# scholarsmate/omega-match

Measured on NVIDIA B200. Metric: haystack_throughput, higher is better.
Workload: dtype u8

## Files before the change

### omega_match_b200/csrc/api.cpp

```cpp
#include <unistd.h>

#include <cstdio>
#include <cstdlib>
#include <cstring>
#include <exception>
#include <string>
#include <thread>

#include "../../include/olm_b200.h"
#include "engine.h"
#include "host_util.h"
#include "multi.h"
#include "store.h"

#ifndef OLM_B200_VERSION
#define OLM_B200_VERSION "0.1.0"
#endif

struct olm_cuda_comm {
  olm::Comm *comm = nullptr;
};

struct omega_list_matcher_struct {
  olm::Engine *engine = nullptr;
// ... 328 lines not shown
int olm_cuda_comm_unique_id(void *id, size_t id_bytes) { return olm::comm_unique_id(id, id_bytes); }

olm_cuda_comm_t *olm_cuda_comm_create(const omega_list_matcher_t *m, const void *id, int rank, int world) {
  if (!m || !m->engine || m->multi) return nullptr;
  olm::Comm *c = olm::comm_create(m->engine, id, rank, world);
  if (!c) return nullptr;
  auto *h = new olm_cuda_comm();
  h->comm = c;
  return h;
}

int olm_cuda_comm_destroy(olm_cuda_comm_t *c) {
  if (!c) return -1;
  olm::comm_destroy(c->comm);
  delete c;
  return 0;
}

int olm_cuda_gather_records(olm_cuda_comm_t *c, const void *dev_records, uint64_t count, int root, int no_overlap,
                            olm_cuda_results_t *out) {
  if (!c || !c->comm) return -1;
  return olm::comm_gather(c->comm, dev_records, count, root, no_overlap != 0, out);
}

int olm_store_inspect(const char *compiled_file, olm_store_info_t *out) {
  if (!compiled_file || !out) return -1;
  size_t n = 0;
  uint8_t *f = olm::map_whole_file(compiled_file, &n, false);
  if (!f) return -1;
  olm::StoreView v;
  const std::string err = olm::parse_store(f, n, &v);
  int rc = -1;
  if (err.empty()) try {
    olm::StagedStore s;
    olm::FilterBudget b;
    const std::string e2 = olm::stage_store(v, b, &s);
    olm::StagedStats ss;
    if (e2.empty() && olm::check_staged_store(v, s) == 0 && olm::stage_stats(v, &ss).empty()) {
      out->flags = v.hdr.flags;
      out->smallest = v.hdr.smallest;
      out->largest = v.hdr.largest;
      out->stored_patterns = v.hdr.stored_patterns;
      out->table_size = v.hdr.table_size;
      out->occupied_buckets = v.hdr.occupied;
      out->len1 = v.n1;
      out->len2 = v.n2;
      out->len3 = v.n3;
      out->len4 = v.n4;
      out->store_bytes = v.hdr.store_bytes;
      out->file_bytes = n;
      out->gram_keys = s.n_keys;
      out->key_bytes = s.params.key_bytes;
      out->key_buckets = s.params.key_mask + 1;
      out->g4_bits = s.params.g4_words * 32;
      out->class_run = s.params.cls.run;
      out->class_and_mask = s.params.cls.and_mask;
      out->class_ranges = s.params.cls.n_ranges;
      for (int i = 0; i < 2; ++i) {
        out->class_lo[i] = s.params.cls.lo[i];
        out->class_hi[i] = s.params.cls.hi[i];
      }
      rc = 0;
    } else {
      std::fprintf(stderr, "libomega_match(b200): %s: %s\n", compiled_file, e2.empty() ? "self check failed" : e2.c_str());
    }
  } catch (const std::exception &ex) {
    std::fprintf(stderr, "libomega_match(b200): %s: malformed store (%s)\n", compiled_file, ex.what());
    rc = -1;
  } else {
    std::fprintf(stderr, "libomega_match(b200): %s: %s\n", compiled_file, err.c_str());
  }
  olm::unmap(f, n);
  return rc;
}

}
```

### omega_match_b200/csrc/device_tables.h

```cpp
#pragma once
#include <cstdint>
#include <vector_types.h>

namespace olm {

struct alignas(16) Slot {
  uint32_t w0;
  uint32_t w1;
  uint32_t meta;
  uint32_t ref;
};
constexpr uint32_t kSlotShort4 = 1u << 31;
constexpr uint32_t kSlotMulti = 1u << 30;
constexpr uint32_t kSlotValueMask = (1u << 30) - 1;

struct alignas(16) Rec {
  uint32_t w0;
  uint32_t len;
  uint32_t store_off;
  uint32_t w1;
};

constexpr uint32_t kHashMul = 0x9E3779B1u;
constexpr uint32_t kHashMul2 = 0x85EBCA6Bu;

#if defined(__CUDACC__)
__host__ __device__
#endif
inline uint32_t key_hash(uint32_t gram, uint32_t tail) { return (gram * kHashMul) ^ (tail * kHashMul2); }

struct ByteClass {
  uint32_t run = 0;
  uint32_t and_mask = 0;
  uint32_t n_ranges = 0;
  uint32_t lo[2] = {0, 0}, hi[2] = {0, 0};
  uint32_t and4 = 0, addlo[2] = {0, 0}, addhi[2] = {0, 0};
};

struct DeviceStore {
  const uint4 *keys = nullptr;
  const Slot *slots = nullptr;
  const Rec *recs = nullptr;
  const uint8_t *store = nullptr;
  const uint32_t *g4 = nullptr;
  const uint32_t *p23 = nullptr;
  const uint32_t *set3 = nullptr;
  const uint32_t *bitmap2 = nullptr;
  uint32_t bitmap1[8] = {0};
  uint32_t key_shift = 32;
  uint32_t key_mask = 0;
  uint32_t empty_key = 0;
  uint32_t key_bytes = 4;
  uint32_t tail_mask = 0;
  uint32_t g4_shift = 32, g4_words = 0;
  uint32_t p23_and = 0, p23_mul = 1, p23_shift = 32, p23_words = 0;
  const uint32_t *sx = nullptr;
  uint32_t sx_words = 0, sx3_shift = 32;
  uint32_t set3_mask = 0;
  uint32_t n_long = 0, n1 = 0, n2 = 0, n3 = 0, n4 = 0;
  uint32_t smallest = 0, largest = 0;
  uint32_t flags = 0;
  uint32_t max_recs = 0;
  uint32_t coop = 0;
  ByteClass cls;
};
#ifndef OLM_COOP_MIN
#define OLM_COOP_MIN 4
#endif
constexpr uint32_t kCoopMinRecs = OLM_COOP_MIN;

}
```

### omega_match_b200/csrc/engine.cu

```cuda
#include "engine.h"

#include <algorithm>
#include <atomic>
#include <condition_variable>
#include <cstdio>
#include <cstdlib>
#include <cstring>
#include <memory>
#include <mutex>
#include <thread>
#include <vector>

#include <cuda_runtime.h>

#include "filters.cuh"
#include "format.cuh"
#include "scan.cuh"
#include "stats.cuh"
#include "transform.cuh"

namespace olm {

namespace {

// ... 90 lines not shown
  uint64_t host_span = 0;
  omega_match_stats_t span_acc{};
};

namespace {
size_t seg_event_for(const EngineImpl &E, uint64_t bytes) {
  if (E.seg_events.size() <= 1 || E.seg_bytes == 0 || bytes == 0) return 0;
  return std::min<size_t>(E.seg_events.size() - 1, size_t((bytes - 1) / E.seg_bytes));
}
int wait_segment(EngineImpl &E, size_t idx) {
  Stager &S = E.stager;
  for (size_t j = std::min(E.seg_waited, idx); j <= idx; ++j) {
    if (S.active) {
      std::unique_lock<std::mutex> lk(S.mu);
      S.cv.wait(lk, [&] { return S.recorded[j] || S.failed.load(); });
      if (S.failed.load()) return -1;
    }
    if (cudaStreamWaitEvent(E.stream, E.seg_events[j], 0) != cudaSuccess) return -1;
  }
  E.seg_waited = std::max(E.seg_waited, idx + 1);
  return 0;
}
}

Engine *Engine::create(const uint8_t *file, size_t size, int device, std::string *err) {
  auto fail = [&](const std::string &m) -> Engine * {
    if (err) *err = m;
    return nullptr;
  };
  StoreView view;
  std::string e = parse_store(file, size, &view);
  if (!e.empty()) return fail(e);

  int ndev = 0;
  if (cudaGetDeviceCount(&ndev) != cudaSuccess || ndev == 0)
    return fail("no CUDA device: this library has no CPU matching path");
  if (device < 0 || device >= ndev) return fail("CUDA device index out of range");
  if (cudaSetDevice(device) != cudaSuccess) return fail("cudaSetDevice failed");
  cudaDeviceProp prop;
  if (cudaGetDeviceProperties(&prop, device) != cudaSuccess) return fail("cudaGetDeviceProperties failed");
  if (prop.major < 10) return fail("this build contains sm_100a code only (needs a B200 class GPU)");

  auto *impl = new EngineImpl();
  Engine *eng = new Engine();
  eng->impl_ = impl;
  impl->device = device;
  impl->sms = prop.multiProcessorCount;
  impl->smem_limit = prop.sharedMemPerBlockOptin;
  impl->hdr = view.hdr;

  StagedStore staged;
  FilterBudget budget;
  const bool has_p23 = view.n1 || view.n2 || view.n3;
  budget.g4_max_log2 = (has_p23 || (view.hdr.flags & kFlagAnyTransform)) ? 19 : OLM_G4_MAX_LOG2;
  budget.p23_max_log2 = 18;
  e = stage_store(view, budget, &staged);
  if (e.empty() && check_staged_store(view, staged) != 0) e = "internal error: staged store failed its self check";
  if (!e.empty()) {
    delete eng;
    return fail(e);
  }
  impl->has_short_234 = view.n2 || view.n3 || view.n4;
  impl->ds = staged.params;
  bool ok = true;
  ok = ok && upload(impl->d_keys, staged.keys, &impl->ds.keys) == 0;
  ok = ok && upload(impl->d_slots, staged.slots, &impl->ds.slots) == 0;
  ok = ok && upload(impl->d_recs, staged.recs, &impl->ds.recs) == 0;
  ok = ok && upload(impl->d_store, staged.store, &impl->ds.store) == 0;
  ok = ok && upload(impl->d_g4, staged.g4, &impl->ds.g4) == 0;
  ok = ok && upload(impl->d_p23, staged.p23, &impl->ds.p23) == 0;
  if (impl->ds.sx_words) ok = ok && upload(impl->d_sx, staged.sx, &impl->ds.sx) == 0;
  ok = ok && upload(impl->d_set3, staged.set3, &impl->ds.set3) == 0;
  ok = ok && upload(impl->d_bitmap2, staged.bitmap2, &impl->ds.bitmap2) == 0;
  if (const char *sp = std::getenv("OLM_HOST_SPAN_BYTES")) {
    const unsigned long long v = std::strtoull(sp, nullptr, 10);
    impl->host_span = (v + kWindowBytes - 1) / kWindowBytes * kWindowBytes;
  }
  {
    StagedStats ss;
    e = stage_stats(view, &ss);
    if (!e.empty()) {
      delete eng;
      return fail(e);
    }
    impl->stats.bloom_mask = ss.bloom_mask;
    impl->stats.map_shift = ss.map_shift;
    impl->stats.map_mask = ss.map_mask;
    impl->stats.largest = view.hdr.largest;
    ok = ok && upload(impl->d_bloom, ss.bloom, &impl->stats.bloom) == 0;
    ok = ok && upload(impl->d_smap, ss.map, &impl->stats.map) == 0;
    ok = ok && upload(impl->d_slens, ss.lens, &impl->stats.lens) == 0;
  }
  ok = ok && cudaStreamCreateWithFlags(&impl->stream, cudaStreamNonBlocking) == cudaSuccess;
  ok = ok && cudaStreamCreateWithFlags(&impl->copy_stream, cudaStreamNonBlocking) == cudaSuccess;
  for (auto &ev : impl->ev) ok = ok && cudaEventCreate(&ev) == cudaSuccess;
  ok = ok && scan_configure(impl->smem_limit) == cudaSuccess;
  impl->geo = scan_pick_geometry(impl->ds, impl->smem_limit);
  if (impl->ds.sx_words) {
    DeviceStore plain = impl->ds;
    plain.sx_words = 0;
    const ScanGeometry g0 = scan_pick_geometry(plain, impl->smem_limit);
    const char *env = std::getenv("OLM_SHORT_LOOK");
    const bool plain_store = !(impl->hdr.flags & kFlagAnyTransform) && !impl->ds.coop;
    const bool weak_p23 = plain_store && (env ? std::atoi(env) != 0 : impl->ds.p23_mul == 1);
    const bool room = impl->geo.stages != 0 && (impl->geo.stages >= g0.stages || impl->geo.stages >= 8) &&
                      impl->geo.chunk_cap >= std::min<uint32_t>(g0.chunk_cap, 256);
    if (!weak_p23 || !room) {
// ... 642 lines not shown
```

### omega_match_b200/csrc/scan.cu

```cuda
#include "scan.cuh"

#include <cstddef>
#include <cstdio>

#include "olm_classes.h"
#include "olm_format.h"
#include "scan_device.cuh"

namespace olm {

namespace {

using namespace dev;

#ifndef OLM_FAST_UNROLL
#define OLM_FAST_UNROLL 2
#endif
#ifndef OLM_GRAB
#define OLM_GRAB 1
#endif
constexpr uint32_t kGrab = OLM_GRAB;
static_assert(kGrab >= 1 && kTileChunks % kGrab == 0, "a grab stays inside one tile");
#ifndef OLM_TICKET_BATCH
#define OLM_TICKET_BATCH 4
// ... 164 lines not shown
      c = T.tail;
    }
    if (fl & kWordBoundary) {
      if (L == 1) {
        if (inside && is_word_byte(c)) return false;
      } else if (is_word_byte(c)) {
        return false;
      }
    }
    if ((fl & kWordSuffix) && inside && is_word_byte(c)) return false;
    if ((fl & kLineEnd) && inside && !is_line_end_byte(c)) return false;
    return true;
  }

  static constexpr uint32_t kNoSlot = 0xFFFFFFFFu;
  static constexpr uint32_t kCoopMin = kCoopMinRecs;
  struct Probe {
    uint32_t tpos, gram, bucket, flags;
    uint4 kb;
  };

  __device__ __forceinline__ void probe_issue(const TileCtx &T, bool valid, uint32_t tpos, bool cand_g, bool cand_p,
                                              Probe &pr) const {
    pr.tpos = tpos;
    pr.flags = 0;
    pr.gram = 0;
    pr.bucket = 0;
    pr.kb = make_uint4(0, 0, 0, 0);
    uint32_t bad_start = 0;
    if (!valid) return;
    const uint32_t q = T.sb32 + kTilePre + tpos;
    if (fl & (kWordBoundary | kWordPrefix | kLineStart)) {
      const bool at0 = T.first && tpos == 0;
      const uint32_t prev = lds8(q - 1);
      if (fl & kWordBoundary) {
        const bool cw = is_word_byte(lds8(q));
        const bool pw = at0 ? false : is_word_byte(prev);
        if (cw == pw) return;
      }
      bool bad = (fl & kWordPrefix) && !at0 && is_word_byte(prev);
      bad = bad || ((fl & kLineStart) && !at0 && !is_line_end_byte(prev));
      if (bad) {
        if (!((fl & kCountAll) && (cand_p || (cand_g && P.st.n4)))) return;
        bad_start = 8u;
      }
    }
    const uint32_t gram = __byte_perm(lds_le32(q), 0, 0x0123);
    if (SX && cand_p) cand_p = short_look(gram);
    pr.flags = 1u | (cand_p ? 4u : 0u) | bad_start;
    if (HAS_G4 && cand_g && T.rem0 - tpos >= P.st.key_bytes) {
      const uint32_t h = key_hash(gram, P.st.tail_mask ? lds_le32(q + 4) & P.st.tail_mask : 0u);
      pr.gram = h;
      if (HAS_CLS) {
        const uint32_t b = h >> P.st.g4_shift;
        if (!((g4s[b >> 5] >> (b & 31)) & 1u)) return;
      }
      pr.flags |= 2u;
      pr.bucket = h >> P.st.key_shift;
      pr.kb = __ldg(P.st.keys + pr.bucket);
    }
  }

  __device__ __forceinline__ bool probe_key(const Probe &pr, uint32_t *slot) const {
    *slot = kNoSlot;
    if (!(pr.flags & 1u)) return false;
    if (HAS_G4 && (pr.flags & 2u)) {
      const uint32_t gram = pr.gram;
      uint4 kb = pr.kb;
      uint32_t bucket = pr.bucket;
      int place;
      while (true) {
        place = kb.x == gram ? 0 : kb.y == gram ? 1 : kb.z == gram ? 2 : kb.w == gram ? 3 : -1;
        if (place >= 0 || kb.w == P.st.empty_key) break;
        bucket = (bucket + 1) & P.st.key_mask;
        kb = __ldg(P.st.keys + bucket);
      }
      if (place >= 0) *slot = 4 * bucket + (uint32_t)place;
    }
    return *slot != kNoSlot || (HAS_P23 && (pr.flags & 4u));
  }

  template <typename Emit>
  __device__ __forceinline__ void verify(const TileCtx &T, uint32_t tpos, uint32_t slot, const uint4 &s_in, bool cand_p,
                                         bool bad_start, bool coop_done, bool emitted, Emit &&emit) const {
    const uint32_t rem = T.rem0 - tpos;
    const uint32_t q = T.sb32 + kTilePre + tpos;
    const bool longest = fl & kLongestOnly;
    const bool count_all = fl & kCountAll;

    if (HAS_G4 && slot != kNoSlot) {
      const uint4 s = COOP ? s_in : __ldg(reinterpret_cast<const uint4 *>(P.st.slots + slot));
      const uint32_t meta = s.z;
      if (meta != 0 && bad_start) {
        if (meta & kSlotShort4) n_miss += stat_inc;
      } else if (meta != 0) {
        const unsigned long long hay = ((unsigned long long)lds_le32(q + 4) << 32) | lds_le32(q);
        if (meta & kSlotValueMask) {
          n_hits += stat_inc;
          n_long_hits += stat_inc;
        }
        auto head_equal = [&](uint32_t len, uint32_t w0, uint32_t w1) {
          const uint32_t drop = len >= 8 ? 0u : (8u - len) * 8u;
          return ((hay ^ (((unsigned long long)w1 << 32) | w0)) << drop) == 0;
        };
        if (meta & kSlotMulti) {
          const uint32_t cnt = (coop_done || !next_bytes_ok(hay, s.x, s.y)) ? 0u : meta & kSlotValueMask;
          for (uint32_t j = 0; j < cnt; ++j) {
// ... 73 lines not shown
            n_hits += stat_inc;
          } else {
            n_miss += stat_inc;
          }
        }
      }
    }
  }

  static __device__ __forceinline__ uint32_t gather4(uint32_t m) { return __umulhi(m, 0x02040810u) & 0xFu; }

  __device__ __forceinline__ uint32_t class_runs16(const uint4 &v, const uint2 &nx) const {
    const ByteClass &c = P.st.cls;
    const uint32_t w[6] = {v.x, v.y, v.z, v.w, nx.x, nx.y};
    const uint32_t and4 = c.and4, lo0 = c.addlo[0], hi0 = c.addhi[0];
    uint32_t a = 0;
    if (c.n_ranges > 1) {
      const uint32_t lo1 = c.addlo[1], hi1 = c.addhi[1];
#pragma unroll
      for (int i = 0; i < 6; ++i) {
        const uint32_t t = w[i] & and4;
        const uint32_t in = ((t + lo0) & ~(t + hi0)) | ((t + lo1) & ~(t + hi1));
        a |= gather4(in & ~w[i] & 0x80808080u) << (4 * i);
      }
    } else {
#pragma unroll
      for (int i = 0; i < 6; ++i) {
        const uint32_t t = w[i] & and4;
        a |= gather4((t + lo0) & ~(t + hi0) & ~w[i] & 0x80808080u) << (4 * i);
      }
    }
    a &= a >> 1;
    a &= a >> 2;
    a &= a >> (c.run - 4);
    return a & 0xFFFFu;
  }
  __device__ __forceinline__ void stage1(const TileCtx &T, uint32_t lpos, uint32_t &cg, uint32_t &cp) const {
    const uint32_t src = T.sb32 + kTilePre + lpos;
    const uint4 v = lds128(src);
    cg = 0;
    cp = 0;
    if (HAS_CLS) {
      cg = class_runs16(v, lds64(src + 16));
      return;
    }
    const uint2 w45 = lds64(src + 16);
    const uint32_t w[6] = {v.x, v.y, v.z, v.w, w45.x, w45.y};
    const uint32_t tmask = P.st.tail_mask;
#pragma unroll
    for (int k = 0; k < 16; ++k) {
      const uint32_t gram = __byte_perm(w[k >> 2], w[(k >> 2) + 1], 0x0123u + 0x1111u * (k & 3));
      if (HAS_G4) {
        const uint32_t tail = __byte_perm(w[(k >> 2) + 1], w[(k >> 2) + 2 > 5 ? 5 : (k >> 2) + 2], 0x3210u + 0x1111u * (k & 3));
        const uint32_t b = key_hash(gram, tail & tmask) >> P.st.g4_shift;
        cg |= ((g4s[b >> 5] >> (b & 31)) & 1u) << k;
      }
      if (HAS_P23) {
        const uint32_t b = ((gram & P.st.p23_and) * P.st.p23_mul) >> P.st.p23_shift;
        cp |= ((p23s[b >> 5] >> (b & 31)) & 1u) << k;
      }
    }
  }

  template <int MODE>
  __device__ __forceinline__ uint32_t verify_batch(const TileCtx &T, uint32_t q2, uint32_t n, uint32_t lane,
                                                   uint32_t stage, uint32_t used, uint32_t cap, uint32_t cbase,
                                                   unsigned long long out_base, uint32_t *overflow) const {
    bool mine = lane < n;
    const unsigned long long ent = mine ? lds64u(q2 + 8u * lane) : 0ull;
    const uint32_t slot = (uint32_t)ent, hi = (uint32_t)(ent >> 32);
    const uint32_t tpos = hi & 0xFFFFu;
    const bool cand_p = (hi >> 16) & 1u, bad_start = (hi >> 17) & 1u;
    uint32_t at = 0, tot = 0, skip = 0;
    const uint32_t keep = stat_inc;
    bool again;
    uint4 s = make_uint4(0, 0, 0, 0);
    if (COOP && HAS_G4 && mine && slot != kNoSlot) s = __ldg(reinterpret_cast<const uint4 *>(P.st.slots + slot));
    do {
      uint32_t cnt = 0, m0 = 0, m1 = 0, m2 = 0, m3 = 0;
      auto emit = [&](uint32_t len) {
        const uint32_t j = cnt - skip;
        if (j == 0) m0 = len;
        else if (j == 1) m1 = len;
        else if (j == 2) m2 = len;
        else if (j == 3) m3 = len;
        ++cnt;
      };
      bool coop = false, emitted0 = false;
      if (COOP && HAS_G4) {
        coop = mine && s.z != 0 && !bad_start && (s.z & kSlotMulti) && (s.z & kSlotValueMask) >= kCoopMin;
        if (coop) {
          const uint32_t mq = T.sb32 + kTilePre + tpos;
          coop = next_bytes_ok(((unsigned long long)lds_le32(mq + 4) << 32) | lds_le32(mq), s.x, s.y);
        }
        uint32_t todo = __ballot_sync(kFull, coop);
        while (todo) {
          const uint32_t src = __ffs(todo) - 1;
          todo &= todo - 1;
          const uint32_t o_tpos = __shfl_sync(kFull, tpos, src), o_first = __shfl_sync(kFull, s.w, src);
          const uint32_t o_cnt = __shfl_sync(kFull, s.z, src) & kSlotValueMask;
          const uint32_t oq = T.sb32 + kTilePre + o_tpos, o_rem = T.rem0 - o_tpos;
          const unsigned long long hay = ((unsigned long long)lds_le32(oq + 4) << 32) | lds_le32(oq);
          uint32_t ncmp = 0;
          for (uint32_t base = 0; base < o_cnt; base += 32) {
            const bool valid = base + lane < o_cnt;
            uint4 r = make_uint4(0, 0, 0, 0);
            if (valid) r = __ldg(reinterpret_cast<const uint4 *>(P.st.recs + o_first + base + lane));
// ... 102 lines not shown
    for (uint32_t base = 0; base < total; base += 32 * kProbeUnroll) {
      Probe pr[kProbeUnroll];
#pragma unroll
      for (int u = 0; u < kProbeUnroll; ++u) {
        const uint32_t idx = base + u * 32 + lane;
        const bool ok = idx < total;
        const uint32_t e = ok ? lds16(q1 + 2u * idx) : 0u;
        probe_issue(T, ok, cbase + (e & 511u), (e >> 9) & 1u, (e >> 10) & 1u, pr[u]);
      }
#pragma unroll
      for (int u = 0; u < kProbeUnroll; ++u) {
        if (base + u * 32 >= total) break;
        uint32_t slot;
        const bool want = probe_key(pr[u], &slot);
        const uint32_t bal = __ballot_sync(kFull, want);
        if (want)
          sts64u(q2 + 8u * (q2n + __popc(bal & lt)),
                 ((unsigned long long)(pr[u].tpos | ((pr[u].flags & 12u) << 14)) << 32) | slot);
        q2n += __popc(bal);
      }
      __syncwarp();
      const bool last = base + 32 * kProbeUnroll >= total;
      while (q2n >= 32 || (last && q2n)) {
        const uint32_t nb = q2n < 32 ? q2n : 32;
        found += verify_batch<MODE>(T, q2, nb, lane, stage, found, cap, cbase, out_base, overflow);
        const uint32_t rest = q2n - nb;
        const unsigned long long mv0 = lane < rest ? lds64u(q2 + 8u * (32 + lane)) : 0ull;
        const unsigned long long mv1 = 32 + lane < rest ? lds64u(q2 + 8u * (64 + lane)) : 0ull;
        __syncwarp();
        if (lane < rest) sts64u(q2 + 8u * lane, mv0);
        if (32 + lane < rest) sts64u(q2 + 8u * (32 + lane), mv1);
        __syncwarp();
        q2n = rest;
      }
    }
    __syncwarp();
    return found;
  }

  template <int MODE, bool PRED>
  __device__ __forceinline__ uint32_t scan_chunk_fast(const TileCtx &T, uint32_t sb_off, uint32_t g4_off,
                                                      uint32_t p23_off, uint32_t q1_off, uint32_t q2_off,
                                                      uint32_t cbase, uint32_t lane, uint32_t stage, uint32_t cap,
                                                      unsigned long long out_base, uint32_t *overflow) const {
    const uint32_t lpos = cbase + lane * 16;
    const uint32_t src = sb_off + kTilePre + lpos;
    const uint4 v = lds128(src);
    uint32_t cand = 0, cp = 0;
    if (HAS_CLS) {
      cand = class_runs16(v, lds64(src + 16));
    } else {
      const uint2 w45 = lds64(src + 16);
      const uint32_t w[6] = {v.x, v.y, v.z, v.w, w45.x, w45.y};
      const uint32_t sh = P.st.g4_shift, tmask = P.st.tail_mask;
      const uint32_t pand = P.st.p23_and, pmul = P.st.p23_mul, psh = P.st.p23_shift;
#pragma unroll
      for (int k = 0; k < 16; ++k) {
        const uint32_t gram = __byte_perm(w[k >> 2], w[(k >> 2) + 1], 0x0123u + 0x1111u * (k & 3));
        if (HAS_G4) {
          uint32_t hk = gram * kHashMul;
          if (!HAS_P23) {
            const uint32_t tail = __byte_perm(w[(k >> 2) + 1], w[(k >> 2) + 2 > 5 ? 5 : (k >> 2) + 2], 0x3210u + 0x1111u * (k & 3));
            hk ^= (tail & tmask) * kHashMul2;
          }
          const uint32_t b = hk >> sh;
          const uint32_t word = lds32(g4_off + ((b >> 5) << 2));
          cand |= ((word >> (b & 31)) & 1u) << k;
        }
        if (HAS_P23) {
          const uint32_t b = ((gram & pand) * pmul) >> psh;
          const uint32_t word = lds32(p23_off + ((b >> 5) << 2));
          cp |= ((word >> (b & 31)) & 1u) << k;
        }
      }
    }
    const uint32_t rem_c = T.rem0 - cbase;
    const uint32_t kbytes = P.st.key_bytes;
    if (rem_c < (uint32_t)kChunkBytes + 8u) {
      const uint32_t fit = rem_c >= kbytes ? rem_c - kbytes + 1u : 0u, lrel = lane * 16;
      cand &= lrel >= fit ? 0u : (fit - lrel >= 16u ? 0xFFFFu : ((1u << (fit - lrel)) - 1u));
    }
    const uint32_t cg = cand;
    cand |= cp;
    if (lpos + 16 > T.nscan) cand &= lpos >= T.nscan ? 0u : ((1u << (T.nscan - lpos)) - 1u);
    const uint32_t cnt = __popc(cand);
    uint32_t incl = cnt;
#pragma unroll
    for (int d = 1; d < 32; d <<= 1) {
      const uint32_t t = __shfl_up_sync(kFull, incl, d);
      if (lane >= (uint32_t)d) incl += t;
    }
    const uint32_t total = __shfl_sync(kFull, incl, 31);
    if (total == 0) return 0;
    {
      uint32_t qa = q1_off + 2u * (incl - cnt);
      if (__any_sync(kFull, cnt > 4)) {
        const uint32_t eb = lane * 16;
#pragma unroll
        for (int k = 0; k < 16; ++k)
          if ((cand >> k) & 1u) {
            uint32_t ent = eb + k;
            if (HAS_P23) ent |= (((cg >> k) & 1u) << 9) | (((cp >> k) & 1u) << 10);
            sts16(qa, ent);
            qa += 2;
          }
      } else {
        const uint32_t eb = lane * 16;
        while (cand) {
          const uint32_t k = __ffs(cand) - 1;
          uint32_t ent = eb + k;
          if (HAS_P23) ent |= (((cg >> k) & 1u) << 9) | (((cp >> k) & 1u) << 10);
          sts16(qa, ent);
          cand &= cand - 1;
          qa += 2;
        }
      }
    }
    __syncwarp();
    const uint32_t q2 = q2_off;
    const uint32_t lt = (1u << lane) - 1u;
    const uint32_t tile_off = sb_off + kTilePre + cbase;
    const uint32_t key_shift = P.st.key_shift, g4_shift = P.st.g4_shift, empty = P.st.empty_key;
    const uint4 *keys = P.st.keys;
    const uint32_t tmask = P.st.tail_mask;
    uint32_t found = 0, q2n = 0;
    constexpr int U = OLM_FAST_UNROLL;
    for (uint32_t base = 0; base < total; base += 32 * U) {
      uint32_t e[U], gram[U], bucket[U];
      bool pass[U], shortc[U];
      uint4 kb[U];
#pragma unroll
      for (int u = 0; u < U; ++u) {
        const uint32_t idx = base + u * 32 + lane;
        pass[u] = idx < total;
        e[u] = pass[u] ? lds16(q1_off + 2u * idx) : 0u;
        shortc[u] = false;
        if (HAS_P23) {
          shortc[u] = (e[u] >> 10) & 1u;
          pass[u] = pass[u] && ((e[u] >> 9) & 1u);
          e[u] &= 511u;
        }
        const uint32_t a = tile_off + e[u], a4 = a & ~3u, sh8 = a << 3;
        const uint32_t x0 = lds32(a4), x1 = lds32(a4 + 4);
        const uint32_t gbe = __byte_perm(__funnelshift_r(x0, x1, sh8), 0, 0x0123);
        if (PRED) {
          const bool at0 = T.first && cbase + e[u] == 0;
          const uint32_t prev = lds8(a - 1), cur = gbe >> 24;
          bool ok = true;
          if (fl & kWordBoundary) ok = is_word_byte(cur) != (at0 ? false : is_word_byte(prev));
          if ((fl & kWordPrefix) && !at0 && is_word_byte(prev)) ok = false;
          if ((fl & kLineStart) && !at0 && !is_line_end_byte(prev)) ok = false;
          pass[u] = pass[u] && ok;
          shortc[u] = shortc[u] && ok;
        }
        if (SX && __any_sync(kFull, shortc[u])) shortc[u] = shortc[u] && short_look(gbe);
        uint32_t h = gbe * kHashMul;
        if (tmask) h ^= (__funnelshift_r(x1, lds32(a4 + 8), sh8) & tmask) * kHashMul2;
        gram[u] = h;
        if (HAS_CLS && !OLM_CLS_SKIP_BITMAP) {
          const uint32_t b = h >> g4_shift;
          const uint32_t word = lds32(g4_off + ((b >> 5) << 2));
          pass[u] = pass[u] && ((word >> (b & 31)) & 1u);
        }
        bucket[u] = h >> key_shift;
        if (HAS_G4 && pass[u]) kb[u] = ld_keys(keys + bucket[u]);
      }
      static_assert(U == 2, "Q2 holds 31 + 2 x 32 entries");
#pragma unroll
      for (int u = 0; u < U; ++u) {
        if (u > 0 && base + u * 32 >= total) break;
        const uint32_t g = gram[u];
        bool hit = HAS_G4 && pass[u] && (kb[u].x == g || kb[u].y == g || kb[u].z == g || kb[u].w == g);
        const bool more = HAS_G4 && pass[u] && !hit && kb[u].w != empty;
        if (!__any_sync(kFull, hit || more || (HAS_P23 && shortc[u]))) continue;
        if (HAS_G4 && __any_sync(kFull, more)) {
          while (pass[u] && !hit && kb[u].w != empty) {
            bucket[u] = (bucket[u] + 1) & P.st.key_mask;
            kb[u] = ld_keys(keys + bucket[u]);
            hit = kb[u].x == g || kb[u].y == g || kb[u].z == g || kb[u].w == g;
          }
        }
        const bool want = hit || (HAS_P23 && shortc[u]);
        const uint32_t bal = __ballot_sync(kFull, want);
        if (!bal) continue;
        const uint32_t place = kb[u].y == g ? 1u : kb[u].z == g ? 2u : kb[u].w == g ? 3u : 0u;
        const uint32_t slot = hit ? 4u * bucket[u] + place : kNoSlot;
        const uint32_t hi32 = (cbase + e[u]) | (HAS_P23 && shortc[u] ? 0x10000u : 0u);
        if (want) sts64u(q2 + 8u * (q2n + __popc(bal & lt)), ((unsigned long long)hi32 << 32) | slot);
        q2n += __popc(bal);
      }
      __syncwarp();
      const bool last = base + 32 * U >= total;
      while (q2n >= 32 || (last && q2n)) {
        const uint32_t nb = q2n < 32 ? q2n : 32;
        found += verify_batch<MODE>(T, q2, nb, lane, stage, found, cap, cbase, out_base, overflow);
        const uint32_t rest = q2n - nb;
        const unsigned long long mv0 = lane < rest ? lds64u(q2 + 8u * (32 + lane)) : 0ull;
        const unsigned long long mv1 = 32 + lane < rest ? lds64u(q2 + 8u * (64 + lane)) : 0ull;
        __syncwarp();
        if (lane < rest) sts64u(q2 + 8u * lane, mv0);
        if (32 + lane < rest) sts64u(q2 + 8u * (32 + lane), mv1);
        __syncwarp();
        q2n = rest;
      }
    }
    __syncwarp();
    return found;
  }

  __device__ __forceinline__ void flush_stats(uint32_t lane) const {
    unsigned long long h = n_hits, mi = n_miss, cm = n_cmp, lh = n_long_hits;
#pragma unroll
    for (int d = 16; d > 0; d >>= 1) {
// ... 256 lines not shown
                        priv32, sc.xf32, lane, true, T);
      __syncwarp();
      if (lane == 0) mbar_arrive32(scanned32 + 8u * s);
      cb = 0;
      work = work && T.nscan != 0;
    } else {
      tile_ctx(I, stage_sb, T);
    }
    if (work) {
      if (FAST)
        n = sc.template scan_chunk_fast<kStageMode, FAST == 2>(T, T.sb32, g4_32, p23_32, q1_32, q2_32, cb, lane, stage32, cap, 0, &ovf);
      else
        n = sc.template scan_chunk<kStageMode>(T, cb, lane, stage32, cap, q1_32, q2_32, 0, &ovf);
    }
    __syncwarp();
    if (!priv_mode && lane == 0) mbar_arrive32(scanned32 + 8u * s);
    ovf = __any_sync(kFull, ovf != 0);
    ChunkDesc d;
    d.count = n;
    d.temp_index = 0;
    if (ovf) {
      d.count = n | kChunkOverflow;
      if (lane == 0) *reinterpret_cast<volatile unsigned int *>(P.redo_flag) = 1u;
    } else if (n) {
      if (n > blk_left) {
        const uint32_t want = n > kWarpTempBlock / 2 ? 2 * n : kWarpTempBlock;
        unsigned long long b = 0;
        if (lane == 0) b = atomicAdd(P.temp_count, (unsigned long long)want);
        blk_next = __shfl_sync(kFull, b, 0);
        blk_left = want;
      }
      if (blk_next + n <= P.temp_cap && blk_next + n <= 0xFFFFFFFFull) {
        uint32_t *dst = P.temp + blk_next;
        for (uint32_t i = lane; i < n; i += 32) dst[i] = lds32(stage32 + 4u * i);
      }
      d.temp_index = (uint32_t)blk_next;
      blk_next += n;
      blk_left -= n;
    }
    if (lane == 0)
      *reinterpret_cast<uint2 *>(P.chunk_desc + ((size_t)tile * kTileChunks + ci)) = make_uint2(d.count, d.temp_index);
    __syncwarp();
    }
  }
  sc.flush_stats(lane);
}

constexpr int kRedoStage = kTilePre + kPrivData;
constexpr size_t kRedoRingBytes = ((size_t)kScanWarps * kRedoStage + 127) & ~size_t(127);
template <bool HAS_G4, bool HAS_P23, bool HAS_CLS, bool XF, bool COOP>
__global__ void __launch_bounds__(kScanThreads, 1) redo_kernel(const __grid_constant__ ScanParams P) {
  extern __shared__ __align__(1024) uint8_t smem[];
  if (*P.redo_flag == 0) return;
  const SmemLayout L = carve<HAS_G4, HAS_P23>(smem, P, kRedoRingBytes, 0);
  const uint32_t tid = threadIdx.x, lane = tid & 31, warp = tid >> 5;
  load_filters<HAS_G4, HAS_P23>(L, P, tid, kScanThreads);
  __syncthreads();
  if (warp >= kScanWarps) return;
  Scanner<HAS_G4, HAS_P23, HAS_CLS, XF, COOP> sc(P, L.g4s, L.p23s);
  sc.stat_inc = 0;
  const uint32_t q1_32 = smem_u32(L.q1 + warp * kChunkBytes), q2_32 = smem_u32(L.q2 + warp * kQ2Entries);
  uint8_t *buf = L.ring + (size_t)warp * kRedoStage;
  const uint32_t priv32 = smem_u32(L.priv) + warp * (uint32_t)kPrivBytes;
  if (XF && !(P.flags & kIdentityMap)) sc.xf32 = smem_u32(L.xf) + warp * (uint32_t)kXfRowBytes;
  const uint64_t n_chunks = (uint64_t)P.num_tiles * kTileChunks;
  for (uint64_t c0 = ((uint64_t)blockIdx.x * kScanWarps + warp) * 32; c0 < n_chunks;
       c0 += (uint64_t)gridDim.x * kScanWarps * 32) {
    uint32_t flagged = 0;
    if (c0 + lane < n_chunks) flagged = P.chunk_desc[c0 + lane].count & kChunkOverflow;
    uint32_t todo = __ballot_sync(kFull, flagged != 0);
    while (todo) {
      const uint64_t ch = c0 + (__ffs(todo) - 1);
      todo &= todo - 1;
      const uint32_t tile = (uint32_t)(ch / kTileChunks), ci = (uint32_t)(ch % kTileChunks);
      StageInfo I;
      fill_tile(P, tile, I);
      const uint32_t cbase = ci * kChunkBytes;
      {
        const long long first = I.boff + cbase - kTilePre;
        uint32_t have = I.staged - cbase;
        if (have > (uint32_t)kPrivData) have = kPrivData;
        for (uint32_t i = lane; i < have + kTilePre; i += 32) buf[i] = first + (long long)i >= 0 ? P.buf[first + (long long)i] : 0;
      }
      __syncwarp();
      TileCtx T;
      build_chunk<XF>(P, I, smem_u32(buf) + kTilePre, cbase, I.boff + (long long)cbase >= (long long)kTilePre ? (uint32_t)kTilePre : 0u,
                      priv32, sc.xf32, lane, false, T);
      unsigned long long base = P.span_base[ch / kPrefixSpan];
      {
        const uint64_t s0 = ch - ch % kPrefixSpan;
        unsigned long long part = 0;
        for (uint64_t j = s0 + lane; j < ch; j += 32) part += P.chunk_desc[j].count & ~kChunkOverflow;
#pragma unroll
        for (int dd = 16; dd > 0; dd >>= 1) part += __shfl_xor_sync(kFull, part, dd);
        base += part;
      }
      if (T.nscan) sc.template scan_chunk<kDirectMode>(T, 0, lane, 0u, 0, q1_32, q2_32, base, nullptr);
      __syncwarp();
    }
  }
}

constexpr int kPrefixThreads = 256;
__global__ void __launch_bounds__(kPrefixThreads) prefix_sum_kernel(const __grid_constant__ ScanParams P) {
  __shared__ unsigned long long s_warp[kPrefixThreads / 32];
  const uint64_t n_chunks = (uint64_t)P.num_tiles * kTileChunks;
  const uint64_t c0 = (uint64_t)blockIdx.x * kPrefixSpan;
  unsigned long long sum = 0;
  for (uint32_t i = threadIdx.x; i < kPrefixSpan; i += kPrefixThreads)
    if (c0 + i < n_chunks) sum += P.chunk_desc[c0 + i].count & ~kChunkOverflow;
#pragma unroll
  for (int d = 16; d > 0; d >>= 1) sum += __shfl_xor_sync(kFull, sum, d);
// ... 39 lines not shown
  const uint64_t c0 = (uint64_t)blockIdx.x * kPrefixSpan;
  constexpr uint32_t kPer = kPrefixSpan / kPrefixThreads;
  uint32_t cnt[kPer];
  uint32_t mine = 0;
#pragma unroll
  for (uint32_t i = 0; i < kPer; ++i) {
    const uint64_t ch = c0 + (uint64_t)tid * kPer + i;
    cnt[i] = ch < n_chunks ? (P.chunk_desc[ch].count & ~kChunkOverflow) : 0u;
    mine += cnt[i];
  }
  uint32_t incl = mine;
#pragma unroll
  for (int d = 1; d < 32; d <<= 1) {
    const uint32_t t = __shfl_up_sync(kFull, incl, d);
    if (lane >= (uint32_t)d) incl += t;
  }
  if (lane == 31) s_warp[warp] = incl;
  __syncthreads();
  uint32_t run = incl - mine;
  for (uint32_t w = 0; w < warp; ++w) run += (uint32_t)s_warp[w];
#pragma unroll
  for (uint32_t i = 0; i < kPer; ++i) {
    s_pre[tid * kPer + i] = run;
    run += cnt[i];
  }
  __syncthreads();
  const unsigned long long span0 = P.span_base[blockIdx.x];
  for (uint32_t g0 = warp * 32; g0 < kPrefixSpan; g0 += (kPrefixThreads / 32) * 32) {
    const uint64_t ch = c0 + g0 + lane;
    uint2 d = make_uint2(0, 0);
    if (ch < n_chunks) d = *reinterpret_cast<const uint2 *>(P.chunk_desc + ch);
    uint32_t todo = __ballot_sync(kFull, d.x != 0 && !(d.x & kChunkOverflow));
    while (todo) {
      const uint32_t src = __ffs(todo) - 1;
      todo &= todo - 1;
      const uint32_t n = __shfl_sync(kFull, d.x, src);
      const unsigned long long tb = __shfl_sync(kFull, d.y, src);
      if (tb + n > P.temp_cap) continue;
      const uint64_t chs = c0 + g0 + src;
      const unsigned long long base = span0 + s_pre[g0 + src];
      const unsigned long long cb = tile_gbase(P, (uint32_t)(chs / kTileChunks)) + (chs % kTileChunks) * kChunkBytes;
      for (uint32_t i = lane; i < n; i += 32) {
        const uint32_t e = __ldg(P.temp + tb + i);
        const unsigned long long r = base + i;
        if (r < P.out_cap) put_record(P, r, cb + (e >> kPackLenBits), e & ((1u << kPackLenBits) - 1));
      }
    }
  }
}

bool store_normalises(const DeviceStore &st) { return st.flags & (kFlagIgnorePunct | kFlagElideSpace); }

size_t redo_smem_bytes(const DeviceStore &st) {
  return kSmemHeader + kRedoRingBytes + size_t(st.g4_words) * 4 + size_t(st.p23_words) * 4 + size_t(st.sx_words) * 4 + kQ2Bytes + kQ1Bytes +
         size_t(kScanWarps) * kPrivBytes + (store_normalises(st) ? size_t(kScanWarps) * kXfRowBytes : 0);
}

template <bool G, bool Q, bool C, bool XF, bool COOP>
cudaError_t launch_variant(const ScanParams &p, int sms, size_t smem, cudaStream_t stream) {
  const int grid = (int)(p.num_tiles < (uint32_t)sms ? p.num_tiles : (uint32_t)sms);
  constexpr bool can_fast = G || Q;
  const int mode = !can_fast || (p.flags & kCountAll) ? 0 : (p.flags & (kWordBoundary | kWordPrefix | kLineStart)) ? 2 : 1;
  bool launched = false;
  if constexpr (Q && !XF && !COOP) {
    if (p.st.sx_words) {
      if (mode == 2)
        scan_kernel<G, Q, C, 2, XF, COOP, true><<<grid, kScanThreads, smem, stream>>>(p);
      else if (mode == 1)
        scan_kernel<G, Q, C, 1, XF, COOP, true><<<grid, kScanThreads, smem, stream>>>(p);
      else
        scan_kernel<G, Q, C, 0, XF, COOP, true><<<grid, kScanThreads, smem, stream>>>(p);
      launched = true;
    }
  }
  if (launched) {
  } else if (mode == 0) {
    scan_kernel<G, Q, C, 0, XF, COOP><<<grid, kScanThreads, smem, stream>>>(p);
  } else if constexpr (can_fast) {
    if (mode == 2)
      scan_kernel<G, Q, C, 2, XF, COOP><<<grid, kScanThreads, smem, stream>>>(p);
    else
      scan_kernel<G, Q, C, 1, XF, COOP><<<grid, kScanThreads, smem, stream>>>(p);
  }
  cudaError_t e = cudaGetLastError();
  if (e != cudaSuccess) return e;
  const uint64_t n_chunks = (uint64_t)p.num_tiles * kTileChunks;
  const uint32_t n_spans = (uint32_t)((n_chunks + kPrefixSpan - 1) / kPrefixSpan);
  prefix_sum_kernel<<<n_spans, kPrefixThreads, 0, stream>>>(p);
  if ((e = cudaGetLastError()) != cudaSuccess) return e;
  prefix_scan_kernel<<<1, 1024, 0, stream>>>(p, n_spans);
  if ((e = cudaGetLastError()) != cudaSuccess) return e;
  place_kernel<<<n_spans, kPrefixThreads, 0, stream>>>(p);
  if ((e = cudaGetLastError()) != cudaSuccess) return e;
  redo_kernel<G, Q, C, XF, COOP><<<grid, kScanThreads, redo_smem_bytes(p.st), stream>>>(p);
  return cudaGetLastError();
}
template <bool G, bool Q, bool C, bool XF>
cudaError_t launch_variant(const ScanParams &p, int sms, size_t smem, cudaStream_t stream) {
  if constexpr (G && !C) {
    if (p.st.coop) return launch_variant<G, Q, C, XF, true>(p, sms, smem, stream);
  }
  return launch_variant<G, Q, C, XF, false>(p, sms, smem, stream);
}
template <bool G, bool Q, bool C>
cudaError_t launch_variant(const ScanParams &p, int sms, size_t smem, cudaStream_t stream) {
  if (p.flags & kWindowMode) return launch_variant<G, Q, C, true>(p, sms, smem, stream);
  return launch_variant<G, Q, C, false>(p, sms, smem, stream);
// ... 79 lines not shown
```

### omega_match_b200/csrc/store.cpp

```cpp
#include "store.h"

#include <algorithm>
#include <cstdlib>

#include "host_util.h"

#ifndef OLM_KEY_EXTRA_LOG2
#define OLM_KEY_EXTRA_LOG2 1
#endif
namespace olm {

std::string parse_store(const uint8_t *f, size_t size, StoreView *v) {
  *v = StoreView{};
  if (!f || size < kHeaderBytes) return "file shorter than the 72-byte header";
  if (std::memcmp(f, kMagicHeader, 8) != 0) return "header magic mismatch";
  Header &h = v->hdr;
  h.version = rd32(f + 8);
  h.flags = rd32(f + 12);
  h.store_bytes = rd64(f + 16);
  h.stored_patterns = rd32(f + 24);
  h.smallest = rd32(f + 28);
  h.largest = rd32(f + 32);
  h.bloom_bytes = rd32(f + 36);
  h.blob_bytes = rd32(f + 40);
// ... 167 lines not shown
      }
      members[group_of_slot[si]].push_back(i);
    }
  }
  uint64_t n_multi = 0;
  for (const auto &m : members)
    if (m.size() > 1) n_multi += m.size();
  if (n_multi > kSlotValueMask) return "too many patterns";
  s->recs.reserve(n_multi);
  for (size_t g = 0; g < members.size(); ++g) {
    Slot &sl = s->slots[slot_of_group[g]];
    const auto &m = members[g];
    if (m.size() == 1) {
      const Pat &p = pats[m[0]];
      sl.meta = p.len;
      sl.ref = uint32_t(p.off);
      sl.w0 = word_of(p.off, p.len, 0);
      sl.w1 = word_of(p.off, p.len, 4);
    } else {
      sl.meta = kSlotMulti | uint32_t(m.size());
      d.max_recs = std::max<uint32_t>(d.max_recs, uint32_t(m.size()));
      sl.ref = uint32_t(s->recs.size());
      const size_t first = s->recs.size();
      for (uint32_t i : m) {
        const Pat &p = pats[i];
        s->recs.push_back(Rec{word_of(p.off, p.len, 0), p.len, uint32_t(p.off), word_of(p.off, p.len, 4)});
      }
      std::stable_sort(s->recs.begin() + first, s->recs.end(), [](const Rec &x, const Rec &y) { return x.len > y.len; });
      const uint32_t K = d.key_bytes;
      uint32_t m0 = 0, m1 = 0;
      bool all0 = K < 8, all1 = K + 1 < 8;
      for (uint32_t i : m) {
        const Pat &p = pats[i];
        if (p.len > K) m0 |= 1u << (s->store[p.off + K] & 31);
        else all0 = false;
        if (p.len > K + 1) m1 |= 1u << (s->store[p.off + K + 1] & 31);
        else all1 = false;
      }
      sl.w0 = all0 ? m0 : 0xFFFFFFFFu;
      sl.w1 = all1 ? m1 : 0xFFFFFFFFu;
    }
  }
  for (uint32_t i = 0; i < v.n4; ++i) {
    bool fresh = false;
    Slot &sl = s->slots[find_or_claim(key_hash(rd32(v.arr4 + 4ull * i), 0), &fresh)];
    sl.meta |= kSlotShort4;
  }
  s->n_keys = uint32_t(n_keys_total);
  d.coop = d.max_recs >= kCoopMinRecs && n_long >= 4 * n_keys_total ? 1u : 0u;
  if (s->recs.empty()) s->recs.push_back(Rec{0, 0, 0, 0});

  if (s->n_keys) {
    const uint32_t n_keys = s->n_keys;
    const uint32_t lg = std::min(budget.g4_max_log2, std::max<uint32_t>(10, ceil_log2(uint64_t(n_keys) * 16)));
    d.g4_shift = 32 - lg;
    d.g4_words = (1u << lg) / 32;
    s->g4.assign(d.g4_words, 0);
    for (const uint4 &kb : s->keys)
      for (uint32_t k : {kb.x, kb.y, kb.z, kb.w})
        if (k != d.empty_key) {
          const uint32_t b = g4_bit(d, k);
          s->g4[b >> 5] |= 1u << (b & 31);
        }
  }

  d.n1 = v.n1;
  d.n2 = v.n2;
  d.n3 = v.n3;
  d.n4 = v.n4;
  if (v.n1 || v.n2 || v.n3) {
    const uint64_t hashed_entries = uint64_t(v.n3) + uint64_t(v.n2) * 256;
    const bool hashed = v.n1 == 0 && hashed_entries * 16 <= (1ull << budget.p23_max_log2);
    if (hashed) {
      const uint32_t lg = std::min(budget.p23_max_log2, std::max<uint32_t>(10, ceil_log2(hashed_entries * 16)));
      d.p23_and = 0xFFFFFF00u;
      d.p23_mul = kHashMul;
      d.p23_shift = 32 - lg;
      d.p23_words = (1u << lg) / 32;
    } else {
      d.p23_and = 0xFFFF0000u;
      d.p23_mul = 1;
      d.p23_shift = 16;
      d.p23_words = 65536 / 32;
    }
    s->p23.assign(d.p23_words, 0);
    auto set_bit = [&](uint32_t gram) {
      const uint32_t b = p23_bit(d, gram);
      s->p23[b >> 5] |= 1u << (b & 31);
    };
    for (uint32_t i = 0; i < v.n3; ++i) set_bit(rd32(v.arr3 + 4ull * i) << 8);
    for (uint32_t w = 0; w < 65536; ++w) {
      if (!(v.bitmap2[w >> 3] & (1u << (w & 7)))) continue;
      if (hashed)
        for (uint32_t c = 0; c < 256; ++c) set_bit((w << 16) | (c << 8));
      else
        set_bit(w << 16);
    }
    if (!hashed)
      for (uint32_t b0 = 0; b0 < 256; ++b0)
        if (v.bitmap1[b0 >> 3] & (1u << (b0 & 7)))
          for (uint32_t b1 = 0; b1 < 256; ++b1) set_bit((b0 << 24) | (b1 << 16));
  }

  {
    const uint32_t lg = std::max<uint32_t>(4, ceil_log2(std::max<uint64_t>(1, uint64_t(v.n3) * 2)));
    d.set3_mask = (1u << lg) - 1;
    s->set3.assign(size_t(1) << lg, 0);
    for (uint32_t i = 0; i < v.n3; ++i) {
      const uint32_t k = rd32(v.arr3 + 4ull * i);
// ... 238 lines not shown
```

### omega_match_b200/csrc/store.h

```cpp
#pragma once
#include <cstddef>
#include <cstdint>
#include <string>
#include <vector>

#include "device_tables.h"
#include "olm_format.h"

namespace olm {

struct StoreView {
  const uint8_t *base = nullptr;
  size_t size = 0;
  Header hdr;
  const uint8_t *patterns = nullptr;
  uint32_t bloom_bits = 0;
  const uint8_t *bloom = nullptr;
  const uint8_t *index = nullptr;
  const uint8_t *blob = nullptr;
  const uint8_t *bitmap1 = nullptr, *bitmap2 = nullptr;
  uint32_t n1 = 0, n2 = 0, n3 = 0, n4 = 0;
  const uint8_t *arr3 = nullptr, *arr4 = nullptr;
};

std::string parse_store(const uint8_t *file, size_t size, StoreView *out);

struct StagedStore {
  std::vector<uint4> keys;
  std::vector<Slot> slots;
  std::vector<Rec> recs;
  std::vector<uint8_t> store;
  std::vector<uint32_t> g4, p23, set3, bitmap2, sx;
  DeviceStore params;
  uint32_t n_keys = 0;
};

struct FilterBudget {
#ifndef OLM_G4_MAX_LOG2
#define OLM_G4_MAX_LOG2 20
#endif
  uint32_t g4_max_log2 = OLM_G4_MAX_LOG2;
  uint32_t p23_max_log2 = 18;
};

std::string stage_store(const StoreView &v, const FilterBudget &budget, StagedStore *out);

struct StagedStats {
  std::vector<unsigned long long> bloom;
  uint32_t bloom_mask = 0;
  std::vector<uint2> map;
  uint32_t map_shift = 32, map_mask = 0;
  std::vector<uint32_t> lens;
};
std::string stage_stats(const StoreView &v, StagedStats *out);

uint64_t check_staged_store(const StoreView &v, const StagedStore &s);

inline uint32_t key_home(const DeviceStore &d, uint32_t key) { return key >> d.key_shift; }
inline uint32_t g4_bit(const DeviceStore &d, uint32_t key) { return key >> d.g4_shift; }
constexpr uint32_t kSx3Off = 2048;
inline uint32_t sx3_bit(const DeviceStore &d, uint32_t key3) { return (key3 * kHashMul) >> d.sx3_shift; }
inline uint32_t p23_bit(const DeviceStore &d, uint32_t gram) {
  return ((gram & d.p23_and) * d.p23_mul) >> d.p23_shift;
}
inline bool class_has(const ByteClass &c, uint32_t b) {
  if (b >= 0x80) return false;
  const uint32_t t = b & c.and_mask;
  for (uint32_t i = 0; i < c.n_ranges; ++i)
    if (t >= c.lo[i] && t <= c.hi[i]) return true;
  return false;
}
inline uint32_t set3_home(const DeviceStore &d, uint32_t key3) { return (key3 * kHashMul >> 8) & d.set3_mask; }

}
```

Measured before the change: 630.8.

## Size gram filter by byte budget with multiply-high indexing; read it from global in redo

The g4 gram bitmap no longer has to be a power of two. Its bit index is now computed with a multiply-high over an arbitrary bit count, and its size is capped by a byte budget (128 KiB by default, 64 KiB when short patterns or transforms are present) rather than a log2 limit. That allows a larger filter that still fits in shared memory, which should cut false-positive candidates. The redo kernel stops copying g4 into shared memory and reads it directly from global memory, which shrinks its shared footprint. In exchange, each probe pays a umulhi instead of a shift, and redo probes go to global memory.

```diff
diff --git a/omega_match_b200/csrc/api.cpp b/omega_match_b200/csrc/api.cpp
--- a/omega_match_b200/csrc/api.cpp
+++ b/omega_match_b200/csrc/api.cpp
@@ -404,7 +404,7 @@
       out->gram_keys = s.n_keys;
       out->key_bytes = s.params.key_bytes;
       out->key_buckets = s.params.key_mask + 1;
-      out->g4_bits = s.params.g4_words * 32;
+      out->g4_bits = s.params.g4_bits;
       out->class_run = s.params.cls.run;
       out->class_and_mask = s.params.cls.and_mask;
       out->class_ranges = s.params.cls.n_ranges;
diff --git a/omega_match_b200/csrc/device_tables.h b/omega_match_b200/csrc/device_tables.h
--- a/omega_match_b200/csrc/device_tables.h
+++ b/omega_match_b200/csrc/device_tables.h
@@ -29,6 +29,17 @@
 #endif
 inline uint32_t key_hash(uint32_t gram, uint32_t tail) { return (gram * kHashMul) ^ (tail * kHashMul2); }
 
+#if defined(__CUDACC__)
+__host__ __device__
+#endif
+inline uint32_t g4_bit_of(uint32_t h, uint32_t bits) {
+#if defined(__CUDA_ARCH__)
+  return __umulhi(h, bits);
+#else
+  return uint32_t((uint64_t(h) * bits) >> 32);
+#endif
+}
+
 struct ByteClass {
   uint32_t run = 0;
   uint32_t and_mask = 0;
@@ -52,7 +63,7 @@
   uint32_t empty_key = 0;
   uint32_t key_bytes = 4;
   uint32_t tail_mask = 0;
-  uint32_t g4_shift = 32, g4_words = 0;
+  uint32_t g4_bits = 0, g4_words = 0;
   uint32_t p23_and = 0, p23_mul = 1, p23_shift = 32, p23_words = 0;
   const uint32_t *sx = nullptr;
   uint32_t sx_words = 0, sx3_shift = 32;
diff --git a/omega_match_b200/csrc/engine.cu b/omega_match_b200/csrc/engine.cu
--- a/omega_match_b200/csrc/engine.cu
+++ b/omega_match_b200/csrc/engine.cu
@@ -166,7 +166,7 @@
   StagedStore staged;
   FilterBudget budget;
   const bool has_p23 = view.n1 || view.n2 || view.n3;
-  budget.g4_max_log2 = (has_p23 || (view.hdr.flags & kFlagAnyTransform)) ? 19 : OLM_G4_MAX_LOG2;
+  if (has_p23 || (view.hdr.flags & kFlagAnyTransform)) budget.g4_max_bytes = 64u << 10;
   budget.p23_max_log2 = 18;
   e = stage_store(view, budget, &staged);
   if (e.empty() && check_staged_store(view, staged) != 0) e = "internal error: staged store failed its self check";
diff --git a/omega_match_b200/csrc/scan.cu b/omega_match_b200/csrc/scan.cu
--- a/omega_match_b200/csrc/scan.cu
+++ b/omega_match_b200/csrc/scan.cu
@@ -240,7 +240,7 @@
       const uint32_t h = key_hash(gram, P.st.tail_mask ? lds_le32(q + 4) & P.st.tail_mask : 0u);
       pr.gram = h;
       if (HAS_CLS) {
-        const uint32_t b = h >> P.st.g4_shift;
+        const uint32_t b = g4_bit_of(h, P.st.g4_bits);
         if (!((g4s[b >> 5] >> (b & 31)) & 1u)) return;
       }
       pr.flags |= 2u;
@@ -420,7 +420,7 @@
       const uint32_t gram = __byte_perm(w[k >> 2], w[(k >> 2) + 1], 0x0123u + 0x1111u * (k & 3));
       if (HAS_G4) {
         const uint32_t tail = __byte_perm(w[(k >> 2) + 1], w[(k >> 2) + 2 > 5 ? 5 : (k >> 2) + 2], 0x3210u + 0x1111u * (k & 3));
-        const uint32_t b = key_hash(gram, tail & tmask) >> P.st.g4_shift;
+        const uint32_t b = g4_bit_of(key_hash(gram, tail & tmask), P.st.g4_bits);
         cg |= ((g4s[b >> 5] >> (b & 31)) & 1u) << k;
       }
       if (HAS_P23) {
@@ -629,7 +629,7 @@
     } else {
       const uint2 w45 = lds64(src + 16);
       const uint32_t w[6] = {v.x, v.y, v.z, v.w, w45.x, w45.y};
-      const uint32_t sh = P.st.g4_shift, tmask = P.st.tail_mask;
+      const uint32_t g4_bits = P.st.g4_bits, tmask = P.st.tail_mask;
       const uint32_t pand = P.st.p23_and, pmul = P.st.p23_mul, psh = P.st.p23_shift;
 #pragma unroll
       for (int k = 0; k < 16; ++k) {
@@ -640,7 +640,7 @@
             const uint32_t tail = __byte_perm(w[(k >> 2) + 1], w[(k >> 2) + 2 > 5 ? 5 : (k >> 2) + 2], 0x3210u + 0x1111u * (k & 3));
             hk ^= (tail & tmask) * kHashMul2;
           }
-          const uint32_t b = hk >> sh;
+          const uint32_t b = g4_bit_of(hk, g4_bits);
           const uint32_t word = lds32(g4_off + ((b >> 5) << 2));
           cand |= ((word >> (b & 31)) & 1u) << k;
         }
@@ -697,7 +697,7 @@
     const uint32_t q2 = q2_off;
     const uint32_t lt = (1u << lane) - 1u;
     const uint32_t tile_off = sb_off + kTilePre + cbase;
-    const uint32_t key_shift = P.st.key_shift, g4_shift = P.st.g4_shift, empty = P.st.empty_key;
+    const uint32_t key_shift = P.st.key_shift, g4_bits = P.st.g4_bits, empty = P.st.empty_key;
     const uint4 *keys = P.st.keys;
     const uint32_t tmask = P.st.tail_mask;
     uint32_t found = 0, q2n = 0;
@@ -735,7 +735,7 @@
         if (tmask) h ^= (__funnelshift_r(x1, lds32(a4 + 8), sh8) & tmask) * kHashMul2;
         gram[u] = h;
         if (HAS_CLS && !OLM_CLS_SKIP_BITMAP) {
-          const uint32_t b = h >> g4_shift;
+          const uint32_t b = g4_bit_of(h, g4_bits);
           const uint32_t word = lds32(g4_off + ((b >> 5) << 2));
           pass[u] = pass[u] && ((word >> (b & 31)) & 1u);
         }
@@ -1098,12 +1098,12 @@
 __global__ void __launch_bounds__(kScanThreads, 1) redo_kernel(const __grid_constant__ ScanParams P) {
   extern __shared__ __align__(1024) uint8_t smem[];
   if (*P.redo_flag == 0) return;
-  const SmemLayout L = carve<HAS_G4, HAS_P23>(smem, P, kRedoRingBytes, 0);
+  const SmemLayout L = carve<false, HAS_P23>(smem, P, kRedoRingBytes, 0);
   const uint32_t tid = threadIdx.x, lane = tid & 31, warp = tid >> 5;
-  load_filters<HAS_G4, HAS_P23>(L, P, tid, kScanThreads);
+  load_filters<false, HAS_P23>(L, P, tid, kScanThreads);
   __syncthreads();
   if (warp >= kScanWarps) return;
-  Scanner<HAS_G4, HAS_P23, HAS_CLS, XF, COOP> sc(P, L.g4s, L.p23s);
+  Scanner<HAS_G4, HAS_P23, HAS_CLS, XF, COOP> sc(P, P.st.g4, L.p23s);
   sc.stat_inc = 0;
   const uint32_t q1_32 = smem_u32(L.q1 + warp * kChunkBytes), q2_32 = smem_u32(L.q2 + warp * kQ2Entries);
   uint8_t *buf = L.ring + (size_t)warp * kRedoStage;
@@ -1249,7 +1249,7 @@
 bool store_normalises(const DeviceStore &st) { return st.flags & (kFlagIgnorePunct | kFlagElideSpace); }
 
 size_t redo_smem_bytes(const DeviceStore &st) {
-  return kSmemHeader + kRedoRingBytes + size_t(st.g4_words) * 4 + size_t(st.p23_words) * 4 + size_t(st.sx_words) * 4 + kQ2Bytes + kQ1Bytes +
+  return kSmemHeader + kRedoRingBytes + size_t(st.p23_words) * 4 + size_t(st.sx_words) * 4 + kQ2Bytes + kQ1Bytes +
          size_t(kScanWarps) * kPrivBytes + (store_normalises(st) ? size_t(kScanWarps) * kXfRowBytes : 0);
 }
 
diff --git a/omega_match_b200/csrc/store.cpp b/omega_match_b200/csrc/store.cpp
--- a/omega_match_b200/csrc/store.cpp
+++ b/omega_match_b200/csrc/store.cpp
@@ -243,9 +243,11 @@
 
   if (s->n_keys) {
     const uint32_t n_keys = s->n_keys;
-    const uint32_t lg = std::min(budget.g4_max_log2, std::max<uint32_t>(10, ceil_log2(uint64_t(n_keys) * 16)));
-    d.g4_shift = 32 - lg;
-    d.g4_words = (1u << lg) / 32;
+    const uint64_t want = 1ull << std::max<uint32_t>(10, ceil_log2(uint64_t(n_keys) * 16));
+    const uint64_t room = uint64_t(budget.g4_max_bytes / 128) * 1024;
+    if (room == 0) return "no shared memory left for the gram filter";
+    d.g4_bits = uint32_t(std::min(want, room));
+    d.g4_words = d.g4_bits / 32;
     s->g4.assign(d.g4_words, 0);
     for (const uint4 &kb : s->keys)
       for (uint32_t k : {kb.x, kb.y, kb.z, kb.w})
diff --git a/omega_match_b200/csrc/store.h b/omega_match_b200/csrc/store.h
--- a/omega_match_b200/csrc/store.h
+++ b/omega_match_b200/csrc/store.h
@@ -36,10 +36,10 @@
 };
 
 struct FilterBudget {
-#ifndef OLM_G4_MAX_LOG2
-#define OLM_G4_MAX_LOG2 20
+#ifndef OLM_G4_MAX_BYTES
+#define OLM_G4_MAX_BYTES (128u << 10)
 #endif
-  uint32_t g4_max_log2 = OLM_G4_MAX_LOG2;
+  uint32_t g4_max_bytes = OLM_G4_MAX_BYTES;
   uint32_t p23_max_log2 = 18;
 };
 
@@ -57,7 +57,7 @@
 uint64_t check_staged_store(const StoreView &v, const StagedStore &s);
 
 inline uint32_t key_home(const DeviceStore &d, uint32_t key) { return key >> d.key_shift; }
-inline uint32_t g4_bit(const DeviceStore &d, uint32_t key) { return key >> d.g4_shift; }
+inline uint32_t g4_bit(const DeviceStore &d, uint32_t key) { return g4_bit_of(key, d.g4_bits); }
 constexpr uint32_t kSx3Off = 2048;
 inline uint32_t sx3_bit(const DeviceStore &d, uint32_t key3) { return (key3 * kHashMul) >> d.sx3_shift; }
 inline uint32_t p23_bit(const DeviceStore &d, uint32_t gram) {
```

Result: no change. 627.9, median of 6 (-0.5%).
